# magenta/ddsp

Hardware: AMD Instinct MI355X
Metric: Msamples/s (Harmonic+FilteredNoise, 16kHz, 100 harmonics) (higher is better)
Workload: dtype f32 (Harmonic wavetables and the FilteredNoise FIR/IR products: 22-bit operands - fp16 hi/lo pairs on the MFMA matrix cores - with fp32 accumulation; everything else plain fp32, the frame phase prefix fp64)

## Files before the change

ddsp_amd/csrc/filtered_noise_mfma.hip:

```cpp
#include <hip/hip_runtime.h>
#include <hip/hip_ext.h>
#include <stdint.h>
#include <cstdlib>
#include <type_traits>
#include "../../include/ddsp_amd.h"
#include "common.h"
#include "split_f16.h"
#include "noise_ir65.h"
#include "profile.h"
#include "filtered_noise_mfma.h"
#include "noise_mfma_plan.h"
#include "launch.h"

namespace ddsp {

constexpr int kMfWaves = 8;
constexpr int kMfPW = kMfWaves / 2;
constexpr int kMfRows = 8 * kMfPW;
static_assert(kMfRows == kMfPlanTileFrames, "noise_mfma_plan.h plans tiles of kMfRows staged frames");
constexpr int kMfTapRowBytes = 17 * 16;
constexpr int kMfTapPlane = kMfRows * kMfTapRowBytes;
constexpr int kMfXStride = 80;
constexpr int kMfXElems = 16 + kMfRows * kMfXStride + 16;
constexpr int kMfXPairs = kMfXElems / 2 + 1;
constexpr int kMfXPlane = kMfWaves == 16 ? 10336 : 5216;
static_assert(kMfXPlane >= kMfXPairs * 4 && kMfXPlane % 16 == 0 && (2 * kMfXPlane / 4) % 32 == 16, "noise plane layout");
constexpr int kMfXOGen = kMfXPlane + 96;
static_assert(kMfXOGen % 16 == 0 && (kMfXOGen / 4) % 32 == 16 && kMfWaves == 8, "noise plane layout, generated noise");
enum class MfNoise { Supplied, Gen11, Gen23 };
template <MfNoise SRC> struct MfX {
  static constexpr bool LO = SRC != MfNoise::Gen11;
  static constexpr int O = LO ? 2 * kMfXPlane : kMfXOGen;
  static constexpr int BYTES = LO ? 4 * kMfXPlane : kMfXOGen + kMfXPlane;
};
struct MfHandoff {
  uint4 frag[kMfPW / 2][4][64];
  float last[kMfRows];
  float tap32[kMfRows];
};

struct MfArgs {
  int N, F, start, scale, fs;
  float inv_fs;
  float bias;
  uint32_t k0, k1;
  uint64_t batch_offset;
  int run_len, run_frames, runs_per_row, n_runs, n_whole;
  FastDiv run_len_div, whole_per_row_div, fs_div;
  const float* x_absmax;
};

static __constant__ Ir65Frags kIr65Frags = make_ir65_frags();

__device__ __forceinline__ void mf_put4(unsigned char* hrow, int t0, float v0, float v1, float v2, float v3) {
  _Float16 h0, l0, h1, l1, h2, l2, h3, l3;
  split(v0, h0, l0); split(v1, h1, l1); split(v2, h2, l2); split(v3, h3, l3);
  unsigned char* q = hrow + t0 * 2;
  *reinterpret_cast<uint2*>(q) = make_uint2(pack(h0, h1), pack(h2, h3));
  *reinterpret_cast<uint2*>(q + kMfTapPlane) = make_uint2(pack(l0, l1), pack(l2, l3));
}
__device__ __forceinline__ void mf_put4_down(unsigned char* hrow, int t1, bool first, float v0, float v1, float v2, float v3) {
  _Float16 h0, l0, h1, l1, h2, l2, h3, l3;
  split(v0, h0, l0); split(v1, h1, l1); split(v2, h2, l2); split(v3, h3, l3);
  unsigned char* q = hrow + (t1 - 3) * 2;
  *reinterpret_cast<uint16_t*>(q) = __builtin_bit_cast(uint16_t, h3);
  *reinterpret_cast<uint16_t*>(q + kMfTapPlane) = __builtin_bit_cast(uint16_t, l3);
  *reinterpret_cast<uint32_t*>(q + 2) = pack(h2, h1);
  *reinterpret_cast<uint32_t*>(q + kMfTapPlane + 2) = pack(l2, l1);
  if (first) {
    *reinterpret_cast<uint16_t*>(q + 6) = __builtin_bit_cast(uint16_t, h0);
    *reinterpret_cast<uint16_t*>(q + kMfTapPlane + 6) = __builtin_bit_cast(uint16_t, l0);
  }
}

template <bool LO>
__device__ __forceinline__ void mf_put_quad(float4 v, int qd, unsigned char* s_xe, unsigned char* s_xo) {
  _Float16 h0, l0, h1, l1, h2, l2, h3, l3;
  split(v.w, h0, l0);
  split(v.z, h1, l1);
  split(v.y, h2, l2);
  split(v.x, h3, l3);
  const int s = qd >> 4, j = 4 * (qd & 15);
  const int u0 = 16 + kMfXStride * s + 60 - j;
  *reinterpret_cast<uint2*>(s_xe + u0 * 2) = make_uint2(pack(h0, h1), pack(h2, h3));
  if (LO) *reinterpret_cast<uint2*>(s_xe + kMfXPlane + u0 * 2) = make_uint2(pack(l0, l1), pack(l2, l3));
  unsigned char* po = s_xo + (u0 + 1) * 2;
  *reinterpret_cast<uint16_t*>(po) = __builtin_bit_cast(uint16_t, h0);
  *reinterpret_cast<uint32_t*>(po + 2) = pack(h1, h2);
  *reinterpret_cast<uint16_t*>(po + 6) = __builtin_bit_cast(uint16_t, h3);
  if (LO) {
    *reinterpret_cast<uint16_t*>(po + kMfXPlane) = __builtin_bit_cast(uint16_t, l0);
    *reinterpret_cast<uint32_t*>(po + kMfXPlane + 2) = pack(l1, l2);
    *reinterpret_cast<uint16_t*>(po + kMfXPlane + 6) = __builtin_bit_cast(uint16_t, l3);
  }
}

template <MfNoise SRC, int NLANES>
__device__ __forceinline__ void mf_noise_tile(int ltid, int b, int zs, const float* __restrict__ x, unsigned char* s_xe,
                                              unsigned char* s_xo, const MfArgs& p) {
  int x_exp = 0;
  if constexpr (SRC == MfNoise::Supplied) x_exp = pow2_exponent(p.x_absmax[b]);
  if constexpr (SRC == MfNoise::Gen11) {
    static_assert((8 * kMfRows) % NLANES == 0, "octets per lane");
#pragma unroll
    for (int h = 0; h < 8 * kMfRows / NLANES; ++h) {
      const int oc = ltid + NLANES * h;
      const int i = zs + 8 * oc;
      float4 v0 = make_float4(0.f, 0.f, 0.f, 0.f), v1 = v0;
      if (i >= 0 && i < p.N) {
        const U4 r = noise_philox(U4{(uint32_t)(i >> 3), (uint32_t)(p.batch_offset + b), 0u, 0u}, p.k0, p.k1);
        v0 = noise_quad(r, 0);
        v1 = noise_quad(r, 1);
        if (i + 7 >= p.N) {
          if (i + 1 >= p.N) v0.y = 0.f;
          if (i + 2 >= p.N) v0.z = 0.f;
          if (i + 3 >= p.N) v0.w = 0.f;
          if (i + 4 >= p.N) v1.x = 0.f;
          if (i + 5 >= p.N) v1.y = 0.f;
          if (i + 6 >= p.N) v1.z = 0.f;
          v1.w = 0.f;
        }
      }
      mf_put_quad<false>(v0, 2 * oc, s_xe, s_xo);
      mf_put_quad<false>(v1, 2 * oc + 1, s_xe, s_xo);
    }
  } else {
    static_assert((16 * kMfRows) % NLANES == 0, "quads per lane");
#pragma unroll
    for (int h = 0; h < 16 * kMfRows / NLANES; ++h) {
      const int qd = ltid + NLANES * h;
      const int i = zs + 4 * qd;
      float4 v = make_float4(0.f, 0.f, 0.f, 0.f);
      if (i >= 0 && i < p.N) {
        if constexpr (SRC == MfNoise::Gen23) {
          v = noise_quad_at((uint32_t)i, p.batch_offset + b, p.k0, p.k1, true);
          if (i + 1 >= p.N) v.y = 0.f;
          if (i + 2 >= p.N) v.z = 0.f;
          if (i + 3 >= p.N) v.w = 0.f;
        } else {
          const float* src = x + (size_t)b * p.N + i;
          if (i + 3 < p.N && ((p.N & 3) == 0)) {
            v = *reinterpret_cast<const float4*>(src);
          } else {
            v.x = src[0];
            if (i + 1 < p.N) v.y = src[1];
            if (i + 2 < p.N) v.z = src[2];
            if (i + 3 < p.N) v.w = src[3];
          }
          if (x_exp) { v.x = ldexpf(v.x, -x_exp); v.y = ldexpf(v.y, -x_exp); v.z = ldexpf(v.z, -x_exp); v.w = ldexpf(v.w, -x_exp); }
        }
      }
      mf_put_quad<true>(v, qd, s_xe, s_xo);
    }
  }
}

template <MfNoise SRC, bool FS64>
__global__ __launch_bounds__(64 * kMfWaves, 4) void noise_mfma65_kernel(
    const float* __restrict__ mag , const float* __restrict__ x ,
    float* __restrict__ ctl_out , float* __restrict__ out , MfArgs p) {
  __shared__ __attribute__((aligned(16))) unsigned char s_taps_all[2][2 * kMfTapPlane];
  constexpr bool GEN_NOISE = SRC == MfNoise::Gen11;
  constexpr bool SUPPLIED = SRC == MfNoise::Supplied;
  constexpr int kXO = MfX<SRC>::O;
  __shared__ __attribute__((aligned(16))) unsigned char s_x_all[2][MfX<SRC>::BYTES];
  __shared__ __attribute__((aligned(16))) std::conditional_t<GEN_NOISE, MfHandoff, uint4> s_hand[2];
  __shared__ __attribute__((aligned(16))) float s_carry[2][kMfPW][128];
  const int tid = threadIdx.x, lane = tid & 63;
  const int wave = __builtin_amdgcn_readfirstlane(tid >> 6);
  const int mi = lane & 15, mg = lane >> 4;
  const int n_my = p.run_len * ((p.n_runs - (int)blockIdx.x + (int)gridDim.x - 1) / (int)gridDim.x);
#define DDSP_MF_TILE(t, b_, zs_, cont_, ffirst_, rel0_)                                                 \
  uint32_t j_, rw_;                                                                                     \
  const int run_ = (int)blockIdx.x + (int)fastdiv((uint32_t)(t), p.run_len_div, j_) * (int)gridDim.x;   \
  const bool last_ = run_ >= p.n_whole;                                                                 \
  const int bq_ = (int)fastdiv((uint32_t)run_, p.whole_per_row_div, rw_);                               \
  const int b_ = last_ ? run_ - p.n_whole : bq_;                                                        \
  const bool cont_ = j_ != 0u;                                                                          \
  const int zs_ = 64 * ((last_ ? p.runs_per_row - 1 : (int)rw_) * p.run_frames + 32 * (int)j_ - 2);     \
  uint32_t fr_;                                                                                         \
  const int fq_ = (int)fastdiv((uint32_t)(zs_ >= 0 ? zs_ : -zs_ + p.fs - 1), p.fs_div, fr_);            \
  const int ffirst_ = (zs_ >= 0) ? fq_ : -fq_;                                                          \
  const int rel0_ = zs_ - ffirst_ * p.fs

  if (wave < kMfPW) {
    constexpr bool HANDOFF = GEN_NOISE;
    const float kLog10 = 2.302585092994046f;
    const bool designer = wave < kMfPW / 2;
    const int rg = wave & (kMfPW / 2 - 1);
    if (designer)
      *reinterpret_cast<uint4*>(s_taps_all[lane >> 5] + (lane & 1) * kMfTapPlane + (16 * rg + ((lane >> 1) & 15)) * kMfTapRowBytes + 256) = make_uint4(0u, 0u, 0u, 0u);
    for (int i = tid; i < 2 * (kMfRows + 1) * 16; i += 64 * kMfPW) {
      unsigned char* const s_xe = s_x_all[i >= (kMfRows + 1) * 16 ? 1 : 0];
      unsigned char* const s_xo = s_xe + kXO;
      const int ii = i >= (kMfRows + 1) * 16 ? i - (kMfRows + 1) * 16 : i;
      const int e = 80 * (ii >> 4) + (ii & 15);
      *reinterpret_cast<uint16_t*>(s_xe + e * 2) = 0;
      *reinterpret_cast<uint16_t*>(s_xo + (e + 1) * 2) = 0;
      if (!GEN_NOISE) {
        *reinterpret_cast<uint16_t*>(s_xe + kMfXPlane + e * 2) = 0;
        *reinterpret_cast<uint16_t*>(s_xo + kMfXPlane + (e + 1) * 2) = 0;
      }
    }
    const int rrow = 16 * rg + mi;
    auto group_unused = [&](int rel0, int zs, int f_first) -> bool {
      if (FS64) return false;
      uint32_t r_;
      const int last_tap_row = (int)fastdiv((uint32_t)(rel0 + 64 * (kMfRows - 1)), p.fs_div, r_);
      const int own_hi = (int)fastdiv((uint32_t)(zs + 64 * kMfRows - 128), p.fs_div, r_) + 2;
      return 16 * rg > last_tap_row && 16 * rg >= own_hi - f_first;
    };
    PackedF4 rq[4];
    float r_last;
    auto fetch_rows = [&](int tick_of_tile) {
      const int t = min(max(tick_of_tile, 0), n_my - 1);
      DDSP_MF_TILE(t, b, zs, cont, f_first, rel0);
      (void)cont;
      if (group_unused(rel0, zs, f_first)) return;
      const int rfr = f_first + rrow;
      const float* __restrict__ src = mag + ((size_t)b * p.F + ((rfr >= 0 && rfr < p.F) ? rfr : 0)) * 65;
#pragma unroll
      for (int c4 = 0; c4 < 4; ++c4) rq[c4] = *reinterpret_cast<const PackedF4*>(src + 16 * mg + 4 * c4);
      r_last = src[64];
    };
    auto scale_rows = [&](int t, f16x8& be_hi, f16x8& be_lo, f16x8& bo_hi, f16x8& bo_lo, float& m_last, float& t32) -> bool {
      DDSP_MF_TILE(t, b, zs, cont, f_first, rel0);
      uint32_t own_r;
      const int own_lo = (zs < 0) ? 0 : (cont ? (int)fastdiv((uint32_t)(zs - 128), p.fs_div, own_r) : f_first) + 2;
      const int own_hi = (int)fastdiv((uint32_t)(zs + 64 * kMfRows - 128), p.fs_div, own_r) + 2;
      const int rfr = f_first + rrow;
      const bool rvalid = rfr >= 0 && rfr < p.F;
      if (f_first + 16 * rg > p.F + 1 || group_unused(rel0, zs, f_first)) return false;
      float y[16];
#pragma unroll
      for (int c4 = 0; c4 < 4; ++c4) { y[4 * c4] = rq[c4].x; y[4 * c4 + 1] = rq[c4].y; y[4 * c4 + 2] = rq[c4].z; y[4 * c4 + 3] = rq[c4].w; }
      m_last = r_last;
      if (p.scale & 1) {
#pragma unroll
        for (int c = 0; c < 16; ++c) y[c] = exp_sigmoid_fast(y[c] + p.bias, kLog10, 2.0f, 1e-7f);
        m_last = exp_sigmoid_fast(m_last + p.bias, kLog10, 2.0f, 1e-7f);
      }
      if (!rvalid) {
#pragma unroll
        for (int c = 0; c < 16; ++c) y[c] = 0.0f;
        m_last = 0.0f;
      }
      if (ctl_out && rvalid && rfr >= own_lo && rfr < own_hi) {
        float* __restrict__ dst = ctl_out + ((size_t)b * p.F + rfr) * 65;
#pragma unroll
        for (int c4 = 0; c4 < 4; ++c4)
          *reinterpret_cast<PackedF4*>(dst + 16 * mg + 4 * c4) = PackedF4{y[4 * c4], y[4 * c4 + 1], y[4 * c4 + 2], y[4 * c4 + 3]};
        if (mg == 0) dst[64] = m_last;
      }
      float ve[8], vo[8];
#pragma unroll
      for (int e = 0; e < 8; ++e) { ve[e] = y[2 * e]; vo[e] = y[2 * e + 1]; }
      split8(ve, be_hi, be_lo);
      split8(vo, bo_hi, bo_lo);
      const float* __restrict__ c32 = kIr65.c + 32 * kIrRowStride + 8 * mg;
      float part = (mg == 0) ? m_last * kIr65.c[32 * kIrRowStride + 32] : 0.0f;
#pragma unroll
      for (int e = 0; e < 8; ++e) part = fmaf(c32[e], ve[e], part);
      part += __shfl_xor(part, 16);
      part += __shfl_xor(part, 32);
      t32 = kIr65.win[32] * part;
      return true;
    };
    auto make_noise = [&](int tick) {
      if (tick >= 0 && tick + 1 < n_my) {
        DDSP_MF_TILE(tick + 1, b, zs, cont, f_first, rel0);
        (void)rel0; (void)f_first; (void)cont;
        unsigned char* const s_xe = s_x_all[(tick + 1) & 1];
        if constexpr (HANDOFF) mf_noise_tile<SRC, 64 * kMfPW>(tid, b, zs, x, s_xe, s_xe + kXO, p);
        else mf_noise_tile<SRC, 32 * kMfPW>(tid - 32 * kMfPW, b, zs, x, s_xe, s_xe + kXO, p);
      }
    };
    if (!designer) {
      if constexpr (HANDOFF) fetch_rows(1);
#pragma unroll 1
      for (int tick = -1; tick < n_my; ++tick) {
        if constexpr (HANDOFF) {
          if (tick + 2 < n_my) {
            MfHandoff& h = s_hand[(tick + 2) & 1];
            f16x8 be_hi, be_lo, bo_hi, bo_lo;
            float m_last, t32;
            if (scale_rows(tick + 2, be_hi, be_lo, bo_hi, bo_lo, m_last, t32)) {
              h.frag[rg][0][lane] = __builtin_bit_cast(uint4, be_hi);
              h.frag[rg][1][lane] = __builtin_bit_cast(uint4, be_lo);
              h.frag[rg][2][lane] = __builtin_bit_cast(uint4, bo_hi);
              h.frag[rg][3][lane] = __builtin_bit_cast(uint4, bo_lo);
              if (mg == 0) { h.last[rrow] = m_last; h.tap32[rrow] = t32; }
            }
          }
          fetch_rows(tick + 3);
        }
        make_noise(tick);
        __syncthreads();
      }
    } else {
      f16x8 afr[2][2][2];
#pragma unroll
      for (int mt = 0; mt < 2; ++mt)
#pragma unroll
        for (int par = 0; par < 2; ++par)
#pragma unroll
          for (int hl = 0; hl < 2; ++hl) {
            const uint4 v = *reinterpret_cast<const uint4*>(kIr65Frags.v[mt][par][hl][lane]);
            afr[mt][par][hl] = frag(v.x, v.y, v.z, v.w);
          }
      auto design_rows = [&](unsigned char* s_taps, const f16x8& be_hi, const f16x8& be_lo, const f16x8& bo_hi,
                             const f16x8& bo_lo, float m_last, float t32) {
          unsigned char* __restrict__ hrow = s_taps + rrow * kMfTapRowBytes;
          const f32x4 zero = {0.f, 0.f, 0.f, 0.f};
#pragma unroll
          for (int mt = 0; mt < 2; ++mt) {
            f32x4 ea = __builtin_amdgcn_mfma_f32_16x16x32_f16(afr[mt][0][0], be_hi, zero, 0, 0, 0);
            f32x4 oa = __builtin_amdgcn_mfma_f32_16x16x32_f16(afr[mt][1][0], bo_hi, zero, 0, 0, 0);
            f32x4 ex = __builtin_amdgcn_mfma_f32_16x16x32_f16(afr[mt][0][0], be_lo, zero, 0, 0, 0);
            f32x4 ox = __builtin_amdgcn_mfma_f32_16x16x32_f16(afr[mt][1][0], bo_lo, zero, 0, 0, 0);
            ex = __builtin_amdgcn_mfma_f32_16x16x32_f16(afr[mt][0][1], be_hi, ex, 0, 0, 0);
            ox = __builtin_amdgcn_mfma_f32_16x16x32_f16(afr[mt][1][1], bo_hi, ox, 0, 0, 0);
            const f32x4 ev = combine(ea, ex), ov = combine(oa, ox);
            const int n0 = 16 * mt + 4 * mg;
            float g0[4], g1[4];
#pragma unroll
            for (int r = 0; r < 4; ++r) {
              const int n = n0 + r;
              const float e = fmaf(m_last, kIr65.c[n * kIrRowStride + 32], ev[r]);
              const float o = ov[r];
              g0[r] = kIr65.win[n] * (e + o);
              g1[r] = (n >= 1) ? kIr65.win[64 - n] * (e - o) : 0.0f;
            }
            mf_put4(hrow, 64 + n0, g0[0], g0[1], g0[2], g0[3]);
            mf_put4(hrow, n0, g1[0], g1[1], g1[2], g1[3]);
            mf_put4_down(hrow, 64 - n0, true, g0[0], g0[1], g0[2], g0[3]);
            mf_put4_down(hrow, 128 - n0, n0 != 0, g1[0], g1[1], g1[2], g1[3]);
          }
          if (mg == 0) {
            _Float16 h, l;
            split(t32, h, l);
            const uint16_t hb = __builtin_bit_cast(uint16_t, h), lb = __builtin_bit_cast(uint16_t, l);
            *reinterpret_cast<uint16_t*>(hrow + 96 * 2) = hb;
            *reinterpret_cast<uint16_t*>(hrow + kMfTapPlane + 96 * 2) = lb;
            *reinterpret_cast<uint16_t*>(hrow + 32 * 2) = hb;
            *reinterpret_cast<uint16_t*>(hrow + kMfTapPlane + 32 * 2) = lb;
          }
      };
      fetch_rows(0);
      auto designer_tick = [&](int tick, auto scale_here_tag) {
        constexpr bool SCALE_HERE = decltype(scale_here_tag)::value;
        if (tick + 1 < n_my) {
          unsigned char* const s_taps = s_taps_all[(tick + 1) & 1];
          if constexpr (SCALE_HERE) {
            f16x8 be_hi, be_lo, bo_hi, bo_lo;
            float m_last = 0.0f, t32 = 0.0f;
            if (scale_rows(tick + 1, be_hi, be_lo, bo_hi, bo_lo, m_last, t32)) design_rows(s_taps, be_hi, be_lo, bo_hi, bo_lo, m_last, t32);
          } else if constexpr (HANDOFF) {
            DDSP_MF_TILE(tick + 1, b, zs, cont, f_first, rel0);
            (void)b; (void)cont;
            if (f_first + 16 * rg <= p.F + 1 && !group_unused(rel0, zs, f_first)) {
              const MfHandoff& h = s_hand[(tick + 1) & 1];
              design_rows(s_taps, __builtin_bit_cast(f16x8, h.frag[rg][0][lane]), __builtin_bit_cast(f16x8, h.frag[rg][1][lane]),
                          __builtin_bit_cast(f16x8, h.frag[rg][2][lane]), __builtin_bit_cast(f16x8, h.frag[rg][3][lane]),
                          h.last[rrow], h.tap32[rrow]);
            }
          }
        }
        if (!HANDOFF) fetch_rows(tick + 2);
        if constexpr (HANDOFF) make_noise(tick);
        __syncthreads();
      };
      designer_tick(-1, std::true_type{});
#pragma unroll 1
      for (int tick = 0; tick < n_my; ++tick) designer_tick(tick, std::integral_constant<bool, !HANDOFF>{});
    }
  } else {
    const int cw = wave - kMfPW;
    const int p_first = 4 * cw;
    f32x4 kept = {0.f, 0.f, 0.f, 0.f};
    float* kept_ot = nullptr;
    long kept_n = 0;
    int kept_exp = 0;
    const int xsel = ((mi & 1) ? 0 : kXO) + 2 * kMfXStride * 2 * p_first;
    const int second = mg >> 1;
    const int u4 = 79 + kMfXStride * second - 16 * 4 - mi + 8 * (mg & 1);
    const int a_base0 = xsel + ((u4 + 1) >> 1) * 4;
    const int q0 = mi - 4 * second;
    const int b_off = (q0 >= 0 && q0 <= 7) ? (2 * q0 + (mg & 1)) * 16 : 256;
    const int b_ptr0 = (2 * p_first + second) * kMfTapRowBytes + b_off;
    const int lane_off = 16 * mi + 4 * mg;
    auto flush_kept = [&](int parity) {
      if (cw >= 1 && kept_ot != nullptr && mi < 8) {
        const float4 cr = *reinterpret_cast<const float4*>(&s_carry[parity][cw - 1][lane_off]);
        float v[4] = {kept[0] + cr.x, kept[1] + cr.y, kept[2] + cr.z, kept[3] + cr.w};
        if constexpr (SUPPLIED) {
#pragma unroll
          for (int r = 0; r < 4; ++r) v[r] = ldexpf(v[r], kept_exp);
        }
#pragma unroll
        for (int r = 0; r < 4; ++r)
          if (kept_n + lane_off + r >= 0 && kept_n + lane_off + r < p.N) kept_ot[lane_off + r] = v[r];
      }
    };
#pragma unroll 1
    for (int tick = -1; tick < n_my; ++tick) {
      if (tick >= 1) flush_kept((tick - 1) & 1);
      if (tick < 0) {
        DDSP_MF_TILE(0, b, zs, cont, f_first, rel0);
        (void)f_first; (void)rel0; (void)cont;
        mf_noise_tile<SRC, 64 * kMfPW>(tid - 64 * kMfPW, b, zs, x, s_x_all[0], s_x_all[0] + kXO, p);
      }
      bool active = false;
      if (tick >= 0) {
        DDSP_MF_TILE(tick, b, zs, cont, f_first, rel0);
        (void)f_first; (void)b; (void)rel0; (void)cont;
        active = (long)zs + 128L * p_first - p.start < (long)p.N;
      }
      if (active) {
        DDSP_MF_TILE(tick, b, zs, cont, f_first, rel0);
        (void)f_first;
        const bool first_direct = cont && cw == 0;
        const unsigned char* const s_taps = s_taps_all[tick & 1];
        const unsigned char* const s_x = s_x_all[tick & 1];
        float* __restrict__ o = out + (size_t)b * p.N;
        const long n_tile = (long)zs + 128L * p_first - p.start;
        const bool interior = n_tile + (first_direct ? 0 : 128) >= 0 && n_tile + 128 * 4 <= (long)p.N && (((p.start | p.N) & 1) == 0);
        float* __restrict__ ot = o + n_tile;
        int o_exp = 0;
        if constexpr (SUPPLIED) o_exp = pow2_exponent(p.x_absmax[b]);
        f32x4 carry = {0.f, 0.f, 0.f, 0.f};
        if (first_direct && mi < 8) {
          const float4 cr = *reinterpret_cast<const float4*>(&s_carry[(tick - 1) & 1][kMfPW - 1][lane_off]);
          carry = (f32x4){cr.x, cr.y, cr.z, cr.w};
        }
        int a_hi[2], a_lo[2], b_ptr = b_ptr0;
        DDSP_KEEP_IN_VGPR(b_ptr);
        __builtin_assume((b_ptr & 15) == 0);
#pragma unroll
        for (int k = 0; k < 2; ++k) {
          a_hi[k] = a_base0 + 640 * k; a_lo[k] = a_base0 + 640 * k + kMfXPlane;
          DDSP_KEEP_IN_VGPR(a_hi[k]);
          DDSP_KEEP_IN_VGPR(a_lo[k]);
          __builtin_assume((a_hi[k] & 3) == 0);
          __builtin_assume((a_lo[k] & 3) == 0);
        }
        f16x8 fah[3], fal[3], fbh_in[2], fbl_in[2], fbh, fbl;
        auto load_step = [&](int j, int slot) {
          const int it = j / 5, c = j - 5 * it;
          const PackedU4 qh = *reinterpret_cast<const PackedU4*>(s_x + a_hi[it >> 1] + 32 * (4 - c) + 2 * kMfXStride * 2 * (it & 1));
          fah[slot] = frag(qh.x, qh.y, qh.z, qh.w);
          if constexpr (!GEN_NOISE) {
            const PackedU4 ql = *reinterpret_cast<const PackedU4*>(s_x + a_lo[it >> 1] + 32 * (4 - c) + 2 * kMfXStride * 2 * (it & 1));
            fal[slot] = frag(ql.x, ql.y, ql.z, ql.w);
          }
          if (c == 0) {
            const unsigned char* tr;
            if (FS64) {
              tr = s_taps + b_ptr + 2 * kMfTapRowBytes * it;
            } else {
              const int P = p_first + it;
              const int row = (int)(((float)(rel0 + 128 * P + 64 * second) + 0.5f) * p.inv_fs);
              tr = s_taps + row * kMfTapRowBytes + b_off;
            }
            fbh_in[it & 1] = *reinterpret_cast<const f16x8*>(tr);
            fbl_in[it & 1] = *reinterpret_cast<const f16x8*>(tr + kMfTapPlane);
          }
        };
        auto column_up = [](f16x8 v) {
          typedef int i32x4 __attribute__((ext_vector_type(4)));
          const i32x4 w = __builtin_bit_cast(i32x4, v);
          i32x4 o;
#pragma unroll
          for (int k = 0; k < 4; ++k) {
            const int t = w[k];
            o[k] = __builtin_amdgcn_update_dpp(0, t, 0x111, 0xF, 0xF, true);
          }
          return __builtin_bit_cast(f16x8, o);
        };
        load_step(0, 0);
        load_step(1, 1);
        load_step(2, 2);
        __builtin_amdgcn_sched_barrier(0);
        f32x4 acc = {0.f, 0.f, 0.f, 0.f}, acc_hl = {0.f, 0.f, 0.f, 0.f}, acc_lh = {0.f, 0.f, 0.f, 0.f};
        auto pipeline = [&](auto interior_tag) {
          constexpr bool kInterior = decltype(interior_tag)::value;
#pragma unroll
          for (int j = 0; j < 20; ++j) {
            const int it = j / 5, c = j - 5 * it, slot = j % 3;
            if (c == 0) { fbh = fbh_in[it & 1]; fbl = fbl_in[it & 1]; }
            acc = __builtin_amdgcn_mfma_f32_16x16x32_f16(fah[slot], fbh, acc, 0, 0, 0);
            acc_hl = __builtin_amdgcn_mfma_f32_16x16x32_f16(fah[slot], fbl, acc_hl, 0, 0, 0);
            if constexpr (!GEN_NOISE) acc_lh = __builtin_amdgcn_mfma_f32_16x16x32_f16(fal[slot], fbh, acc_lh, 0, 0, 0);
            __builtin_amdgcn_sched_barrier(0);
            if (j + 3 < 20) load_step(j + 3, slot);
            if (c < 4) { fbh = column_up(fbh); fbl = column_up(fbl); }
            __builtin_amdgcn_sched_barrier(0);
            if (c == 4) {
              const f32x4 comb = combine(acc, acc_hl + acc_lh) + carry;
              acc = (f32x4){0.f, 0.f, 0.f, 0.f};
              acc_hl = (f32x4){0.f, 0.f, 0.f, 0.f};
              acc_lh = (f32x4){0.f, 0.f, 0.f, 0.f};
              if (it == 0) kept = comb;
              if (mi < 8 && (it > 0 || first_direct)) {
                const int idx = lane_off + 128 * it;
                f32x4 st4 = comb;
                if constexpr (SUPPLIED) {
#pragma unroll
                  for (int r = 0; r < 4; ++r) { const float v = comb[r]; st4[r] = ldexpf(v, o_exp); }
                }
                if (kInterior) {
                  *reinterpret_cast<float2*>(ot + idx) = make_float2(st4[0], st4[1]);
                  *reinterpret_cast<float2*>(ot + idx + 2) = make_float2(st4[2], st4[3]);
                } else {
#pragma unroll
                  for (int r = 0; r < 4; ++r) {
                    const float v = st4[r];
                    if (n_tile + idx + r >= 0 && n_tile + idx + r < p.N) ot[idx + r] = v;
                  }
                }
              }
#pragma unroll
              for (int r = 0; r < 4; ++r) {
                const float v = comb[r];
                carry[r] = __builtin_bit_cast(float, __builtin_amdgcn_update_dpp(0, __builtin_bit_cast(int, v), 0x108, 0xF, 0xF, true));
              }
              if (it == 3 && mi >= 8)
                *reinterpret_cast<float4*>(&s_carry[tick & 1][cw][lane_off - 128]) = make_float4(comb[0], comb[1], comb[2], comb[3]);
            }
          }
        };
        if (interior) pipeline(std::true_type{});
        else pipeline(std::false_type{});
        kept_ot = ot;
        kept_n = n_tile;
        kept_exp = o_exp;
      } else {
        kept_ot = nullptr;
      }
      __syncthreads();
    }
    flush_kept((n_my - 1) & 1);
  }
#undef DDSP_MF_TILE
}

bool noise_mfma65_ok(int F, int M, int N, int padding, const void* noise, int scale) {
  const int frame_size = (N + F - 1) / F;
  return scale != 0 && M == 65 && padding == 0 && frame_size >= 64 && (frame_size % 64) == 0 && frame_size <= 4096 &&
         (N + frame_size - 1) / frame_size == F && (noise == nullptr || (((uintptr_t)noise) & 15) == 0);
}

__global__ __launch_bounds__(1024) void row_absmax_kernel(const float* __restrict__ x, int N, float* __restrict__ out) {
  __shared__ float s_m[16];
  const float* row = x + (size_t)blockIdx.x * N;
  float m = 0.0f;
  for (int i = threadIdx.x; i < N; i += 1024) m = fmaxf(m, fabsf(row[i]));
  m = wave_max_nonneg_dpp(m);
  if ((threadIdx.x & 63) == 0) s_m[threadIdx.x >> 6] = m;
  __syncthreads();
  if (threadIdx.x == 0) {
    float r = 0.0f;
    for (int w = 0; w < 16; ++w) r = fmaxf(r, s_m[w]);
    out[blockIdx.x] = r;
  }
}

int launch_noise_mfma65(const float* magnitudes, const float* noise, float* audio, float* ctl_magnitudes, int B, int F,
                        int N, int start, float initial_bias, int scale, uint64_t seed, uint64_t batch_offset,
                        int bits23, float* row_scratch , hipStream_t st) {
  MfArgs q;
  q.x_absmax = nullptr;
  if (noise) {
    if (!row_scratch) return DDSP_ERR_WORKSPACE;
    hipLaunchKernelGGL(row_absmax_kernel, dim3((unsigned)B), dim3(1024), 0, st, noise, N, row_scratch);
    q.x_absmax = row_scratch;
  }
  q.N = N; q.F = F; q.start = start; q.bias = initial_bias; q.scale = scale;
  q.fs = (N + F - 1) / F; q.inv_fs = 1.0f / (float)q.fs;
  q.k0 = (uint32_t)seed; q.k1 = (uint32_t)(seed >> 32); q.batch_offset = batch_offset;
  q.fs_div = make_fastdiv((uint32_t)q.fs);
  static const int n_cu = [] {
    int dev = 0, v = 0;
    if (hipGetDevice(&dev) != hipSuccess ||
        hipDeviceGetAttribute(&v, hipDeviceAttributeMultiprocessorCount, dev) != hipSuccess || v <= 0)
      v = 256;
    return v;
  }();
  const int slots = n_cu * (kMfWaves == 16 ? 1 : 2);
  struct PlanKey { int B, F, fs, start, slots; };
  static thread_local PlanKey plan_key = {0, 0, 0, 0, 0};
  static thread_local MfRunPlan plan;
  if (plan_key.B != B || plan_key.F != F || plan_key.fs != q.fs || plan_key.start != start || plan_key.slots != slots) {
    plan = plan_noise_mfma_runs(B, F, q.fs, start, slots);
    plan_key = PlanKey{B, F, q.fs, start, slots};
  }
  q.run_len = plan.run_len; q.run_frames = plan.run_frames; q.runs_per_row = plan.runs_per_row;
  q.n_runs = plan.n_runs; q.n_whole = plan.n_whole;
  q.run_len_div = make_fastdiv((uint32_t)plan.run_len);
  q.whole_per_row_div = make_fastdiv((uint32_t)(plan.runs_per_row > 1 ? plan.runs_per_row - 1 : 1));
  const dim3 grid((unsigned)plan.grid);
  hipEvent_t ev0, ev1;
  profile_kernel_events(kNoiseMfma, &ev0, &ev1);
#define DDSP_LAUNCH_MF(SRC, FS64)                                                                                      \
  hipExtLaunchKernelGGL((noise_mfma65_kernel<MfNoise::SRC, FS64>), grid, dim3(64 * kMfWaves), 0, st, ev0, ev1, 0, magnitudes, noise, \
                        ctl_magnitudes, audio, q)
#define DDSP_LAUNCH_MF_SRC(FS64)                                                                                       \
  do { if (noise) DDSP_LAUNCH_MF(Supplied, FS64); else if (bits23) DDSP_LAUNCH_MF(Gen23, FS64); else DDSP_LAUNCH_MF(Gen11, FS64); } while (0)
  if (q.fs == 64) DDSP_LAUNCH_MF_SRC(true); else DDSP_LAUNCH_MF_SRC(false);
#undef DDSP_LAUNCH_MF_SRC
#undef DDSP_LAUNCH_MF
  return check_launch();
}

}
```

ddsp_amd/csrc/noise_mfma_plan.h:

```cpp
#pragma once

namespace ddsp {

constexpr int kMfPlanTileFrames = 32;
constexpr int kMfPlanHistory = 2;
constexpr int kMfPlanTick = 4;

struct MfRunPlan {
  int frames;
  int run_len;
  int run_frames;
  int runs_per_row;
  int n_runs;
  int n_whole;
  int grid;
  int ticks;
  long cost;
};

inline int mf_run_frames(int run_len) { return kMfPlanTileFrames * run_len - kMfPlanHistory; }

inline long mf_run_cost(int len, int out_frames) {
  long c = (long)kMfPlanTick * len;
  int staged = out_frames + kMfPlanHistory;
  for (int j = 0; j < len && staged > 0; ++j, staged -= kMfPlanTileFrames) c += staged < kMfPlanTileFrames ? staged : kMfPlanTileFrames;
  return c;
}

inline MfRunPlan plan_noise_mfma_runs(int B, int F, int frame_size, int start, int slots) {
  MfRunPlan best{};
  const long samples = (long)F * frame_size + start;
  const int frames = (int)((samples + 63) / 64);
  const int max_len = (frames + kMfPlanHistory + kMfPlanTileFrames - 1) / kMfPlanTileFrames;
  int last_rpr = 0;
  for (int len = 1; len <= (max_len > 1 ? max_len : 1); ++len) {
    const int rf = mf_run_frames(len);
    const int rpr = (frames + rf - 1) / rf;
    if (rpr == last_rpr) continue;
    last_rpr = rpr;
    const long n_runs = (long)B * rpr, n_whole = (long)B * (rpr - 1);
    const long grid = n_runs < slots ? n_runs : slots;
    const long whole_cost = mf_run_cost(len, rf), last_cost = mf_run_cost(len, frames - (rpr - 1) * rf);
    long cost = 0;
    for (long i = 0; i < grid; ++i) {
      const long whole = n_whole > i ? (n_whole - i + grid - 1) / grid : 0;
      const long all = (n_runs - i + grid - 1) / grid;
      const long c = whole * whole_cost + (all - whole) * last_cost;
      if (c > cost) cost = c;
    }
    if (best.run_len == 0 || cost <= best.cost) {
      best.frames = frames; best.run_len = len; best.run_frames = rf; best.runs_per_row = rpr;
      best.n_runs = (int)n_runs; best.n_whole = (int)n_whole; best.grid = (int)grid;
      best.ticks = (int)(len * ((n_runs + grid - 1) / grid)); best.cost = cost;
    }
  }
  return best;
}

inline void mf_plan_run(const MfRunPlan& p, int run, int* b, int* r) {
  if (run >= p.n_whole) { *b = run - p.n_whole; *r = p.runs_per_row - 1; }
  else { *b = run / (p.runs_per_row - 1); *r = run % (p.runs_per_row - 1); }
}
struct MfPlanTile { int staged, first_out, cont; };
inline MfPlanTile mf_plan_tile(const MfRunPlan& p, int r, int j) {
  const int staged = r * p.run_frames + kMfPlanTileFrames * j - kMfPlanHistory;
  return MfPlanTile{staged, j ? staged : staged + kMfPlanHistory, j != 0};
}

}
```

ddsp_amd/csrc/split_f16.h:

```cpp
#pragma once
#include <hip/hip_runtime.h>
#include <stdint.h>

namespace ddsp {

typedef _Float16 f16x8 __attribute__((ext_vector_type(8)));
typedef float f32x4 __attribute__((ext_vector_type(4)));
typedef uint32_t u32x4 __attribute__((ext_vector_type(4)));
typedef __fp16 h16x2 __attribute__((ext_vector_type(2)));

constexpr float kLoScale = 2048.0f;

struct __attribute__((packed, aligned(4))) PackedF4 { float x, y, z, w; };
struct __attribute__((packed, aligned(4))) PackedU4 { uint32_t x, y, z, w; };

__device__ __forceinline__ void split(float v, _Float16& hi, _Float16& lo) {
  hi = (_Float16)v;
  lo = (_Float16)((v - (float)hi) * kLoScale);
}
__device__ __forceinline__ void split8(const float (&v)[8], f16x8& hi, f16x8& lo) {
#pragma unroll
  for (int e = 0; e < 8; ++e) {
    _Float16 h, l;
    split(v[e], h, l);
    hi[e] = h;
    lo[e] = l;
  }
}
__device__ __forceinline__ void store_fragment(u32x4* packed, size_t frag_id, int lane, const float (&v)[8]) {
  f16x8 hi, lo;
  split8(v, hi, lo);
  packed[frag_id * 128 + lane] = __builtin_bit_cast(u32x4, hi);
  packed[frag_id * 128 + 64 + lane] = __builtin_bit_cast(u32x4, lo);
}
__device__ __forceinline__ uint32_t pack(_Float16 a, _Float16 b) {
  return (uint32_t)__builtin_bit_cast(uint16_t, a) | ((uint32_t)__builtin_bit_cast(uint16_t, b) << 16);
}
__device__ __forceinline__ f16x8 frag(uint32_t a, uint32_t b, uint32_t c, uint32_t d) {
  const u32x4 v = {a, b, c, d};
  return __builtin_bit_cast(f16x8, v);
}
template <class T>
__device__ __forceinline__ T combine(T acc, T cross) { return acc + cross * (1.0f / kLoScale); }

}
```

Baseline: 119,300.

## Replace per-tick fastdiv tile decoding with incremental tile walker; fast path for Gen23 noise

Adds an incremental MfTileWalker that steps through each block's tiles, updating frame index and remainder by precomputed quotient/remainder deltas. This replaces the DDSP_MF_TILE macro, which recomputed several fast divisions on every tick in every role (fetch, scale, noise, MFMA). Each wave now carries its own walker state in registers. Also adds a Gen23 fast path that skips the per-quad bounds checks when a tile lies entirely inside the signal. The walker has to reproduce the old own_lo/own_hi/tap-row arithmetic exactly, and the extra live tile structs raise register pressure.

```diff
diff --git a/ddsp_amd/csrc/filtered_noise_mfma.hip b/ddsp_amd/csrc/filtered_noise_mfma.hip
--- a/ddsp_amd/csrc/filtered_noise_mfma.hip
+++ b/ddsp_amd/csrc/filtered_noise_mfma.hip
@@ -45,8 +45,7 @@
   float bias;
   uint32_t k0, k1;
   uint64_t batch_offset;
-  int run_len, run_frames, runs_per_row, n_runs, n_whole;
-  FastDiv run_len_div, whole_per_row_div, fs_div;
+  MfWalkPlan wp;
   const float* x_absmax;
 };
 
@@ -126,6 +125,16 @@
     }
   } else {
     static_assert((16 * kMfRows) % NLANES == 0, "quads per lane");
+    if constexpr (SRC == MfNoise::Gen23) {
+      if (zs >= 0 && (long)zs + 64L * kMfRows <= (long)p.N) {
+#pragma unroll
+        for (int h = 0; h < 16 * kMfRows / NLANES; ++h) {
+          const int qd = ltid + NLANES * h;
+          mf_put_quad<true>(noise_quad_at((uint32_t)(zs + 4 * qd), p.batch_offset + b, p.k0, p.k1, true), qd, s_xe, s_xo);
+        }
+        return;
+      }
+    }
 #pragma unroll
     for (int h = 0; h < 16 * kMfRows / NLANES; ++h) {
       const int qd = ltid + NLANES * h;
@@ -169,19 +178,9 @@
   const int tid = threadIdx.x, lane = tid & 63;
   const int wave = __builtin_amdgcn_readfirstlane(tid >> 6);
   const int mi = lane & 15, mg = lane >> 4;
-  const int n_my = p.run_len * ((p.n_runs - (int)blockIdx.x + (int)gridDim.x - 1) / (int)gridDim.x);
-#define DDSP_MF_TILE(t, b_, zs_, cont_, ffirst_, rel0_)                                                 \
-  uint32_t j_, rw_;                                                                                     \
-  const int run_ = (int)blockIdx.x + (int)fastdiv((uint32_t)(t), p.run_len_div, j_) * (int)gridDim.x;   \
-  const bool last_ = run_ >= p.n_whole;                                                                 \
-  const int bq_ = (int)fastdiv((uint32_t)run_, p.whole_per_row_div, rw_);                               \
-  const int b_ = last_ ? run_ - p.n_whole : bq_;                                                        \
-  const bool cont_ = j_ != 0u;                                                                          \
-  const int zs_ = 64 * ((last_ ? p.runs_per_row - 1 : (int)rw_) * p.run_frames + 32 * (int)j_ - 2);     \
-  uint32_t fr_;                                                                                         \
-  const int fq_ = (int)fastdiv((uint32_t)(zs_ >= 0 ? zs_ : -zs_ + p.fs - 1), p.fs_div, fr_);            \
-  const int ffirst_ = (zs_ >= 0) ? fq_ : -fq_;                                                          \
-  const int rel0_ = zs_ - ffirst_ * p.fs
+  const int n_my = MfTileWalker<FS64>::tiles_of_block((int)blockIdx.x, (int)gridDim.x, p.wp);
+  MfTileWalker<FS64> walker;
+  walker.init((int)blockIdx.x, (int)gridDim.x, p.wp, n_my);
 
   if (wave < kMfPW) {
     constexpr bool HANDOFF = GEN_NOISE;
@@ -203,34 +202,25 @@
       }
     }
     const int rrow = 16 * rg + mi;
-    auto group_unused = [&](int rel0, int zs, int f_first) -> bool {
+    auto group_unused = [&](const MfTile& t) -> bool {
       if (FS64) return false;
-      uint32_t r_;
-      const int last_tap_row = (int)fastdiv((uint32_t)(rel0 + 64 * (kMfRows - 1)), p.fs_div, r_);
-      const int own_hi = (int)fastdiv((uint32_t)(zs + 64 * kMfRows - 128), p.fs_div, r_) + 2;
-      return 16 * rg > last_tap_row && 16 * rg >= own_hi - f_first;
+      return 16 * rg > t.last_tap_row && 16 * rg >= t.own_hi - t.f_first;
     };
     PackedF4 rq[4];
     float r_last;
-    auto fetch_rows = [&](int tick_of_tile) {
-      const int t = min(max(tick_of_tile, 0), n_my - 1);
-      DDSP_MF_TILE(t, b, zs, cont, f_first, rel0);
-      (void)cont;
-      if (group_unused(rel0, zs, f_first)) return;
-      const int rfr = f_first + rrow;
-      const float* __restrict__ src = mag + ((size_t)b * p.F + ((rfr >= 0 && rfr < p.F) ? rfr : 0)) * 65;
+    auto fetch_rows = [&](const MfTile& t) {
+      if (group_unused(t)) return;
+      const int rfr = t.f_first + rrow;
+      const float* __restrict__ src = mag + ((size_t)t.b * p.F + ((rfr >= 0 && rfr < p.F) ? rfr : 0)) * 65;
 #pragma unroll
       for (int c4 = 0; c4 < 4; ++c4) rq[c4] = *reinterpret_cast<const PackedF4*>(src + 16 * mg + 4 * c4);
       r_last = src[64];
     };
-    auto scale_rows = [&](int t, f16x8& be_hi, f16x8& be_lo, f16x8& bo_hi, f16x8& bo_lo, float& m_last, float& t32) -> bool {
-      DDSP_MF_TILE(t, b, zs, cont, f_first, rel0);
-      uint32_t own_r;
-      const int own_lo = (zs < 0) ? 0 : (cont ? (int)fastdiv((uint32_t)(zs - 128), p.fs_div, own_r) : f_first) + 2;
-      const int own_hi = (int)fastdiv((uint32_t)(zs + 64 * kMfRows - 128), p.fs_div, own_r) + 2;
-      const int rfr = f_first + rrow;
+    auto scale_rows = [&](const MfTile& t, f16x8& be_hi, f16x8& be_lo, f16x8& bo_hi, f16x8& bo_lo, float& m_last, float& t32) -> bool {
+      const int b = t.b, own_lo = t.own_lo, own_hi = t.own_hi;
+      const int rfr = t.f_first + rrow;
       const bool rvalid = rfr >= 0 && rfr < p.F;
-      if (f_first + 16 * rg > p.F + 1 || group_unused(rel0, zs, f_first)) return false;
+      if (t.f_first + 16 * rg > p.F + 1 || group_unused(t)) return false;
       float y[16];
 #pragma unroll
       for (int c4 = 0; c4 < 4; ++c4) { y[4 * c4] = rq[c4].x; y[4 * c4 + 1] = rq[c4].y; y[4 * c4 + 2] = rq[c4].z; y[4 * c4 + 3] = rq[c4].w; }
@@ -266,25 +256,28 @@
       t32 = kIr65.win[32] * part;
       return true;
     };
-    auto make_noise = [&](int tick) {
+    auto make_noise = [&](int tick, const MfTile& t ) {
       if (tick >= 0 && tick + 1 < n_my) {
-        DDSP_MF_TILE(tick + 1, b, zs, cont, f_first, rel0);
-        (void)rel0; (void)f_first; (void)cont;
         unsigned char* const s_xe = s_x_all[(tick + 1) & 1];
-        if constexpr (HANDOFF) mf_noise_tile<SRC, 64 * kMfPW>(tid, b, zs, x, s_xe, s_xe + kXO, p);
-        else mf_noise_tile<SRC, 32 * kMfPW>(tid - 32 * kMfPW, b, zs, x, s_xe, s_xe + kXO, p);
+        if constexpr (HANDOFF) mf_noise_tile<SRC, 64 * kMfPW>(tid, t.b, t.zs, x, s_xe, s_xe + kXO, p);
+        else mf_noise_tile<SRC, 32 * kMfPW>(tid - 32 * kMfPW, t.b, t.zs, x, s_xe, s_xe + kXO, p);
       }
     };
     if (!designer) {
-      if constexpr (HANDOFF) fetch_rows(1);
+      MfTile n1 = walker.next(p.wp), n2 = n1, n3 = n1;
+      if constexpr (HANDOFF) {
+        n2 = walker.next(p.wp);
+        fetch_rows(n2);
+      }
 #pragma unroll 1
       for (int tick = -1; tick < n_my; ++tick) {
         if constexpr (HANDOFF) {
+          n3 = walker.next(p.wp);
           if (tick + 2 < n_my) {
             MfHandoff& h = s_hand[(tick + 2) & 1];
             f16x8 be_hi, be_lo, bo_hi, bo_lo;
             float m_last, t32;
-            if (scale_rows(tick + 2, be_hi, be_lo, bo_hi, bo_lo, m_last, t32)) {
+            if (scale_rows(n2, be_hi, be_lo, bo_hi, bo_lo, m_last, t32)) {
               h.frag[rg][0][lane] = __builtin_bit_cast(uint4, be_hi);
               h.frag[rg][1][lane] = __builtin_bit_cast(uint4, be_lo);
               h.frag[rg][2][lane] = __builtin_bit_cast(uint4, bo_hi);
@@ -292,10 +285,12 @@
               if (mg == 0) { h.last[rrow] = m_last; h.tap32[rrow] = t32; }
             }
           }
-          fetch_rows(tick + 3);
-        }
-        make_noise(tick);
+          fetch_rows(n3);
+        }
+        make_noise(tick, n1);
         __syncthreads();
+        if constexpr (HANDOFF) { n1 = n2; n2 = n3; }
+        else n1 = walker.next(p.wp);
       }
     } else {
       f16x8 afr[2][2][2];
@@ -346,7 +341,8 @@
             *reinterpret_cast<uint16_t*>(hrow + kMfTapPlane + 32 * 2) = lb;
           }
       };
-      fetch_rows(0);
+      MfTile d1 = walker.next(p.wp);
+      fetch_rows(d1);
       auto designer_tick = [&](int tick, auto scale_here_tag) {
         constexpr bool SCALE_HERE = decltype(scale_here_tag)::value;
         if (tick + 1 < n_my) {
@@ -354,11 +350,9 @@
           if constexpr (SCALE_HERE) {
             f16x8 be_hi, be_lo, bo_hi, bo_lo;
             float m_last = 0.0f, t32 = 0.0f;
-            if (scale_rows(tick + 1, be_hi, be_lo, bo_hi, bo_lo, m_last, t32)) design_rows(s_taps, be_hi, be_lo, bo_hi, bo_lo, m_last, t32);
+            if (scale_rows(d1, be_hi, be_lo, bo_hi, bo_lo, m_last, t32)) design_rows(s_taps, be_hi, be_lo, bo_hi, bo_lo, m_last, t32);
           } else if constexpr (HANDOFF) {
-            DDSP_MF_TILE(tick + 1, b, zs, cont, f_first, rel0);
-            (void)b; (void)cont;
-            if (f_first + 16 * rg <= p.F + 1 && !group_unused(rel0, zs, f_first)) {
+            if (d1.f_first + 16 * rg <= p.F + 1 && !group_unused(d1)) {
               const MfHandoff& h = s_hand[(tick + 1) & 1];
               design_rows(s_taps, __builtin_bit_cast(f16x8, h.frag[rg][0][lane]), __builtin_bit_cast(f16x8, h.frag[rg][1][lane]),
                           __builtin_bit_cast(f16x8, h.frag[rg][2][lane]), __builtin_bit_cast(f16x8, h.frag[rg][3][lane]),
@@ -366,9 +360,11 @@
             }
           }
         }
-        if (!HANDOFF) fetch_rows(tick + 2);
-        if constexpr (HANDOFF) make_noise(tick);
+        const MfTile d2 = walker.next(p.wp);
+        if (!HANDOFF) fetch_rows(d2);
+        if constexpr (HANDOFF) make_noise(tick, d1);
         __syncthreads();
+        d1 = d2;
       };
       designer_tick(-1, std::true_type{});
 #pragma unroll 1
@@ -402,23 +398,19 @@
           if (kept_n + lane_off + r >= 0 && kept_n + lane_off + r < p.N) kept_ot[lane_off + r] = v[r];
       }
     };
+    MfTile cur = walker.next(p.wp);
 #pragma unroll 1
     for (int tick = -1; tick < n_my; ++tick) {
-      if (tick >= 1) flush_kept((tick - 1) & 1);
-      if (tick < 0) {
-        DDSP_MF_TILE(0, b, zs, cont, f_first, rel0);
-        (void)f_first; (void)rel0; (void)cont;
-        mf_noise_tile<SRC, 64 * kMfPW>(tid - 64 * kMfPW, b, zs, x, s_x_all[0], s_x_all[0] + kXO, p);
-      }
-      bool active = false;
-      if (tick >= 0) {
-        DDSP_MF_TILE(tick, b, zs, cont, f_first, rel0);
-        (void)f_first; (void)b; (void)rel0; (void)cont;
-        active = (long)zs + 128L * p_first - p.start < (long)p.N;
-      }
+      if (tick >= 1) {
+        flush_kept((tick - 1) & 1);
+        cur = walker.next(p.wp);
+      }
+      if (tick < 0) mf_noise_tile<SRC, 64 * kMfPW>(tid - 64 * kMfPW, cur.b, cur.zs, x, s_x_all[0], s_x_all[0] + kXO, p);
+      const bool active = tick >= 0 && (long)cur.zs + 128L * p_first - p.start < (long)p.N;
       if (active) {
-        DDSP_MF_TILE(tick, b, zs, cont, f_first, rel0);
-        (void)f_first;
+        const int b = cur.b, zs = cur.zs, rel0 = cur.rel0;
+        const bool cont = cur.cont;
+        (void)rel0;
         const bool first_direct = cont && cw == 0;
         const unsigned char* const s_taps = s_taps_all[tick & 1];
         const unsigned char* const s_x = s_x_all[tick & 1];
@@ -541,7 +533,6 @@
     }
     flush_kept((n_my - 1) & 1);
   }
-#undef DDSP_MF_TILE
 }
 
 bool noise_mfma65_ok(int F, int M, int N, int padding, const void* noise, int scale) {
@@ -578,7 +569,6 @@
   q.N = N; q.F = F; q.start = start; q.bias = initial_bias; q.scale = scale;
   q.fs = (N + F - 1) / F; q.inv_fs = 1.0f / (float)q.fs;
   q.k0 = (uint32_t)seed; q.k1 = (uint32_t)(seed >> 32); q.batch_offset = batch_offset;
-  q.fs_div = make_fastdiv((uint32_t)q.fs);
   static const int n_cu = [] {
     int dev = 0, v = 0;
     if (hipGetDevice(&dev) != hipSuccess ||
@@ -594,10 +584,7 @@
     plan = plan_noise_mfma_runs(B, F, q.fs, start, slots);
     plan_key = PlanKey{B, F, q.fs, start, slots};
   }
-  q.run_len = plan.run_len; q.run_frames = plan.run_frames; q.runs_per_row = plan.runs_per_row;
-  q.n_runs = plan.n_runs; q.n_whole = plan.n_whole;
-  q.run_len_div = make_fastdiv((uint32_t)plan.run_len);
-  q.whole_per_row_div = make_fastdiv((uint32_t)(plan.runs_per_row > 1 ? plan.runs_per_row - 1 : 1));
+  q.wp = mf_walk_plan(plan, q.fs);
   const dim3 grid((unsigned)plan.grid);
   hipEvent_t ev0, ev1;
   profile_kernel_events(kNoiseMfma, &ev0, &ev1);
diff --git a/ddsp_amd/csrc/noise_mfma_plan.h b/ddsp_amd/csrc/noise_mfma_plan.h
--- a/ddsp_amd/csrc/noise_mfma_plan.h
+++ b/ddsp_amd/csrc/noise_mfma_plan.h
@@ -67,4 +67,110 @@
   return MfPlanTile{staged, j ? staged : staged + kMfPlanHistory, j != 0};
 }
 
+#if defined(__HIPCC__)
+#define DDSP_MF_HD __host__ __device__ inline
+#else
+#define DDSP_MF_HD inline
+#endif
+
+struct MfDiv { unsigned d, magic; };
+inline MfDiv mf_make_div(unsigned d) { return MfDiv{d, d <= 1u ? 0xFFFFFFFFu : (unsigned)((1ull << 32) / d)}; }
+DDSP_MF_HD unsigned mf_div(unsigned n, MfDiv f, unsigned* rem) {
+  unsigned q = (unsigned)(((unsigned long long)n * f.magic) >> 32);
+  unsigned r = n - q * f.d;
+  if (r >= f.d) { ++q; r -= f.d; }
+  *rem = r;
+  return q;
 }
+
+struct MfWalkPlan {
+  int run_len, run_frames, runs_per_row, n_runs, n_whole, fs;
+  MfDiv whole_per_row;
+  MfDiv by_fs;
+  int q_tile, r_tile, q_own, r_own, q_tap, r_tap;
+  int low_own;
+};
+inline MfWalkPlan mf_walk_plan(const MfRunPlan& p, int fs) {
+  MfWalkPlan w{};
+  w.run_len = p.run_len; w.run_frames = p.run_frames; w.runs_per_row = p.runs_per_row; w.n_runs = p.n_runs; w.n_whole = p.n_whole;
+  w.fs = fs;
+  w.whole_per_row = mf_make_div((unsigned)(p.runs_per_row > 1 ? p.runs_per_row - 1 : 1));
+  w.by_fs = mf_make_div((unsigned)fs);
+  const int tile = 64 * kMfPlanTileFrames;
+  w.q_tile = tile / fs; w.r_tile = tile % fs;
+  w.q_own = (tile - 128) / fs; w.r_own = (tile - 128) % fs;
+  w.q_tap = (tile - 64) / fs; w.r_tap = (tile - 64) % fs;
+  w.low_own = fs == 64 ? -2 : -1;
+  return w;
+}
+
+struct MfTile {
+  int b;
+  int zs;
+  bool cont;
+  int f_first, rel0;
+  int own_lo, own_hi;
+  int last_tap_row;
+};
+
+template <bool FS64>
+struct MfTileWalker {
+  int run, j, b, zs, f_first, rel0;
+  int left;
+  int grid;
+
+  DDSP_MF_HD static int tiles_of_block(int block, int grid_, const MfWalkPlan& w) {
+    return w.run_len * ((w.n_runs - block + grid_ - 1) / grid_);
+  }
+  DDSP_MF_HD void begin_run(const MfWalkPlan& w) {
+    j = 0;
+    int r;
+    if (run >= w.n_whole) { b = run - w.n_whole; r = w.runs_per_row - 1; }
+    else { unsigned rem; b = (int)mf_div((unsigned)run, w.whole_per_row, &rem); r = (int)rem; }
+    zs = 64 * (r * w.run_frames - kMfPlanHistory);
+    if (FS64) { f_first = zs >> 6; rel0 = 0; }
+    else if (zs >= 0) { unsigned rem; f_first = (int)mf_div((unsigned)zs, w.by_fs, &rem); rel0 = (int)rem; }
+    else { f_first = w.low_own; rel0 = zs - w.low_own * w.fs; }
+  }
+  DDSP_MF_HD void init(int block, int grid_, const MfWalkPlan& w, int n_my) {
+    grid = grid_;
+    run = block;
+    left = n_my;
+    begin_run(w);
+  }
+  DDSP_MF_HD MfTile tile(const MfWalkPlan& w) const {
+    MfTile t;
+    t.b = b; t.zs = zs; t.cont = j != 0;
+    t.f_first = FS64 ? zs >> 6 : f_first;
+    t.rel0 = FS64 ? 0 : rel0;
+    if (FS64) {
+      t.own_hi = t.f_first + 32;
+      t.own_lo = zs < 0 ? 0 : t.f_first + (t.cont ? 0 : 2);
+      t.last_tap_row = 31;
+    } else {
+      t.own_hi = f_first + w.q_own + (rel0 + w.r_own >= w.fs ? 1 : 0) + 2;
+      t.own_lo = zs < 0 ? 0 : f_first + (t.cont && rel0 < 128 ? w.low_own : 0) + 2;
+      t.last_tap_row = w.q_tap + (rel0 + w.r_tap >= w.fs ? 1 : 0);
+    }
+    return t;
+  }
+  DDSP_MF_HD MfTile next(const MfWalkPlan& w) {
+    const MfTile t = tile(w);
+    if (left > 1) {
+      --left;
+      if (++j < w.run_len) {
+        zs += 64 * kMfPlanTileFrames;
+        if (!FS64) {
+          f_first += w.q_tile; rel0 += w.r_tile;
+          if (rel0 >= w.fs) { rel0 -= w.fs; ++f_first; }
+        }
+      } else {
+        run += grid;
+        begin_run(w);
+      }
+    }
+    return t;
+  }
+};
+
+}
```

Result: no change. 120,100, median of 6 (+0.7%).

## Fold hi/lo MFMA products into one accumulator with scaled fp16 splits

Applied to the files above, without the earlier changes.

Tap and noise operands are now pre-scaled by powers of two before the hi/lo fp16 split, and the lo part is no longer rescaled. This lets all partial products share a single fp32 accumulator, with one fmaf applying the output scale and carry at the end. The DPP column shift moves from the two B fragments to the accumulator, and the column loop order is reversed to match. This removes two extra accumulators and the separate combine step, lowering register pressure. In exchange the MFMAs within each step form a serial dependency chain, and small lo values risk fp16 subnormal or precision loss from the new scaling.

```diff
diff --git a/ddsp_amd/csrc/filtered_noise_mfma.hip b/ddsp_amd/csrc/filtered_noise_mfma.hip
--- a/ddsp_amd/csrc/filtered_noise_mfma.hip
+++ b/ddsp_amd/csrc/filtered_noise_mfma.hip
@@ -52,16 +52,34 @@
 
 static __constant__ Ir65Frags kIr65Frags = make_ir65_frags();
 
+constexpr float kMfTapScale = 8192.0f;
+constexpr float kMfNoiseScale = 16384.0f;
+constexpr float kMfOutScale = 1.0f / (kMfTapScale * kMfNoiseScale);
+constexpr double mf_max_tap_gain() {
+  const Ir65Table t = make_ir65_table();
+  double worst = 0.0;
+  for (int n = 0; n <= 32; ++n) {
+    double sum = 0.0;
+    for (int i = 0; i <= 32; ++i) sum += t.c[n * kIrRowStride + i] < 0 ? -(double)t.c[n * kIrRowStride + i] : (double)t.c[n * kIrRowStride + i];
+    for (int i = 0; i < 32; ++i) sum += t.c[n * kIrRowStride + 40 + i] < 0 ? -(double)t.c[n * kIrRowStride + 40 + i] : (double)t.c[n * kIrRowStride + 40 + i];
+    worst = sum > worst ? sum : worst;
+  }
+  return worst;
+}
+static_assert(2.0 * mf_max_tap_gain() * kMfTapScale < 0.5 * 65504.0, "a scaled tap must stay far inside fp16's range");
+
 __device__ __forceinline__ void mf_put4(unsigned char* hrow, int t0, float v0, float v1, float v2, float v3) {
   _Float16 h0, l0, h1, l1, h2, l2, h3, l3;
-  split(v0, h0, l0); split(v1, h1, l1); split(v2, h2, l2); split(v3, h3, l3);
+  split_scaled(v0, kMfTapScale, h0, l0); split_scaled(v1, kMfTapScale, h1, l1);
+  split_scaled(v2, kMfTapScale, h2, l2); split_scaled(v3, kMfTapScale, h3, l3);
   unsigned char* q = hrow + t0 * 2;
   *reinterpret_cast<uint2*>(q) = make_uint2(pack(h0, h1), pack(h2, h3));
   *reinterpret_cast<uint2*>(q + kMfTapPlane) = make_uint2(pack(l0, l1), pack(l2, l3));
 }
 __device__ __forceinline__ void mf_put4_down(unsigned char* hrow, int t1, bool first, float v0, float v1, float v2, float v3) {
   _Float16 h0, l0, h1, l1, h2, l2, h3, l3;
-  split(v0, h0, l0); split(v1, h1, l1); split(v2, h2, l2); split(v3, h3, l3);
+  split_scaled(v0, kMfTapScale, h0, l0); split_scaled(v1, kMfTapScale, h1, l1);
+  split_scaled(v2, kMfTapScale, h2, l2); split_scaled(v3, kMfTapScale, h3, l3);
   unsigned char* q = hrow + (t1 - 3) * 2;
   *reinterpret_cast<uint16_t*>(q) = __builtin_bit_cast(uint16_t, h3);
   *reinterpret_cast<uint16_t*>(q + kMfTapPlane) = __builtin_bit_cast(uint16_t, l3);
@@ -76,10 +94,10 @@
 template <bool LO>
 __device__ __forceinline__ void mf_put_quad(float4 v, int qd, unsigned char* s_xe, unsigned char* s_xo) {
   _Float16 h0, l0, h1, l1, h2, l2, h3, l3;
-  split(v.w, h0, l0);
-  split(v.z, h1, l1);
-  split(v.y, h2, l2);
-  split(v.x, h3, l3);
+  split_scaled(v.w, kMfNoiseScale, h0, l0);
+  split_scaled(v.z, kMfNoiseScale, h1, l1);
+  split_scaled(v.y, kMfNoiseScale, h2, l2);
+  split_scaled(v.x, kMfNoiseScale, h3, l3);
   const int s = qd >> 4, j = 4 * (qd & 15);
   const int u0 = 16 + kMfXStride * s + 60 - j;
   *reinterpret_cast<uint2*>(s_xe + u0 * 2) = make_uint2(pack(h0, h1), pack(h2, h3));
@@ -338,7 +356,7 @@
           }
           if (mg == 0) {
             _Float16 h, l;
-            split(t32, h, l);
+            split_scaled(t32, kMfTapScale, h, l);
             const uint16_t hb = __builtin_bit_cast(uint16_t, h), lb = __builtin_bit_cast(uint16_t, l);
             *reinterpret_cast<uint16_t*>(hrow + 96 * 2) = hb;
             *reinterpret_cast<uint16_t*>(hrow + kMfTapPlane + 96 * 2) = lb;
@@ -444,16 +462,16 @@
           __builtin_assume((a_hi[k] & 3) == 0);
           __builtin_assume((a_lo[k] & 3) == 0);
         }
-        f16x8 fah[3], fal[3], fbh_in[2], fbl_in[2], fbh, fbl;
+        f16x8 fah[3], fal[3], fbh[2], fbl[2];
         auto load_step = [&](int j, int slot) {
-          const int it = j / 5, c = j - 5 * it;
+          const int it = j / 5, c = 4 - j % 5;
           const PackedU4 qh = *reinterpret_cast<const PackedU4*>(s_x + a_hi[it >> 1] + 32 * (4 - c) + 2 * kMfXStride * 2 * (it & 1));
           fah[slot] = frag(qh.x, qh.y, qh.z, qh.w);
           if constexpr (!GEN_NOISE) {
             const PackedU4 ql = *reinterpret_cast<const PackedU4*>(s_x + a_lo[it >> 1] + 32 * (4 - c) + 2 * kMfXStride * 2 * (it & 1));
             fal[slot] = frag(ql.x, ql.y, ql.z, ql.w);
           }
-          if (c == 0) {
+          if (c == 4) {
             const unsigned char* tr;
             if (FS64) {
               tr = s_taps + b_ptr + 2 * kMfTapRowBytes * it;
@@ -462,44 +480,42 @@
               const int row = (int)(((float)(rel0 + 128 * P + 64 * second) + 0.5f) * p.inv_fs);
               tr = s_taps + row * kMfTapRowBytes + b_off;
             }
-            fbh_in[it & 1] = *reinterpret_cast<const f16x8*>(tr);
-            fbl_in[it & 1] = *reinterpret_cast<const f16x8*>(tr + kMfTapPlane);
+            fbh[it & 1] = *reinterpret_cast<const f16x8*>(tr);
+            fbl[it & 1] = *reinterpret_cast<const f16x8*>(tr + kMfTapPlane);
           }
         };
-        auto column_up = [](f16x8 v) {
-          typedef int i32x4 __attribute__((ext_vector_type(4)));
-          const i32x4 w = __builtin_bit_cast(i32x4, v);
-          i32x4 o;
+        auto column_up = [](f32x4 v) {
+          f32x4 o;
 #pragma unroll
           for (int k = 0; k < 4; ++k) {
-            const int t = w[k];
-            o[k] = __builtin_amdgcn_update_dpp(0, t, 0x111, 0xF, 0xF, true);
-          }
-          return __builtin_bit_cast(f16x8, o);
+            const float t = v[k];
+            o[k] = __builtin_bit_cast(float, __builtin_amdgcn_update_dpp(0, __builtin_bit_cast(int, t), 0x111, 0xF, 0xF, true));
+          }
+          return o;
         };
         load_step(0, 0);
         load_step(1, 1);
         load_step(2, 2);
         __builtin_amdgcn_sched_barrier(0);
-        f32x4 acc = {0.f, 0.f, 0.f, 0.f}, acc_hl = {0.f, 0.f, 0.f, 0.f}, acc_lh = {0.f, 0.f, 0.f, 0.f};
+        f32x4 acc = {0.f, 0.f, 0.f, 0.f};
         auto pipeline = [&](auto interior_tag) {
           constexpr bool kInterior = decltype(interior_tag)::value;
 #pragma unroll
           for (int j = 0; j < 20; ++j) {
-            const int it = j / 5, c = j - 5 * it, slot = j % 3;
-            if (c == 0) { fbh = fbh_in[it & 1]; fbl = fbl_in[it & 1]; }
-            acc = __builtin_amdgcn_mfma_f32_16x16x32_f16(fah[slot], fbh, acc, 0, 0, 0);
-            acc_hl = __builtin_amdgcn_mfma_f32_16x16x32_f16(fah[slot], fbl, acc_hl, 0, 0, 0);
-            if constexpr (!GEN_NOISE) acc_lh = __builtin_amdgcn_mfma_f32_16x16x32_f16(fal[slot], fbh, acc_lh, 0, 0, 0);
+            const int it = j / 5, c = 4 - j % 5, slot = j % 3;
+            f32x4 a = {0.f, 0.f, 0.f, 0.f};
+            if (c < 4) a = column_up(acc);
+            a = __builtin_amdgcn_mfma_f32_16x16x32_f16(fah[slot], fbh[it & 1], a, 0, 0, 0);
+            a = __builtin_amdgcn_mfma_f32_16x16x32_f16(fah[slot], fbl[it & 1], a, 0, 0, 0);
+            if constexpr (!GEN_NOISE) a = __builtin_amdgcn_mfma_f32_16x16x32_f16(fal[slot], fbh[it & 1], a, 0, 0, 0);
+            acc = a;
             __builtin_amdgcn_sched_barrier(0);
             if (j + 3 < 20) load_step(j + 3, slot);
-            if (c < 4) { fbh = column_up(fbh); fbl = column_up(fbl); }
             __builtin_amdgcn_sched_barrier(0);
-            if (c == 4) {
-              const f32x4 comb = combine(acc, acc_hl + acc_lh) + carry;
-              acc = (f32x4){0.f, 0.f, 0.f, 0.f};
-              acc_hl = (f32x4){0.f, 0.f, 0.f, 0.f};
-              acc_lh = (f32x4){0.f, 0.f, 0.f, 0.f};
+            if (c == 0) {
+              f32x4 comb;
+#pragma unroll
+              for (int r = 0; r < 4; ++r) { const float v = a[r], cr = carry[r]; comb[r] = __builtin_fmaf(v, kMfOutScale, cr); }
               if (it == 0) kept = comb;
               if (mi < 8 && (it > 0 || first_direct)) {
                 const int idx = lane_off + 128 * it;
diff --git a/ddsp_amd/csrc/split_f16.h b/ddsp_amd/csrc/split_f16.h
--- a/ddsp_amd/csrc/split_f16.h
+++ b/ddsp_amd/csrc/split_f16.h
@@ -17,6 +17,11 @@
 __device__ __forceinline__ void split(float v, _Float16& hi, _Float16& lo) {
   hi = (_Float16)v;
   lo = (_Float16)((v - (float)hi) * kLoScale);
+}
+__device__ __forceinline__ void split_scaled(float v, float s, _Float16& hi, _Float16& lo) {
+  const float t = v * s;
+  hi = (_Float16)t;
+  lo = (_Float16)(t - (float)hi);
 }
 __device__ __forceinline__ void split8(const float (&v)[8], f16x8& hi, f16x8& lo) {
 #pragma unroll
```

Result: faster. 121,100 before, 123,600 after (median of 6 runs) (+2.0%).
